# shenwei356/bio

Measured on AMD Instinct MI355X. Metric: Gbases/s hashed (k=21 ntHash + minimizer), higher is better.
Workload: dtype u64

## Files before the change

bio_amd/csrc/biosketch.hip:

```cpp
#include "host_internal.hpp"
#include "kernels_host.hpp"

extern "C" int bsk_abi_version(void) { return BSK_ABI_VERSION; }

extern "C" const char *bsk_err_name(int e) {
    switch (e) {
        case BSK_OK: return "ok";
        case BSK_ERR_INVALID_K: return "ErrInvalidK";
        case BSK_ERR_EMPTY_SEQ: return "ErrEmptySeq";
        case BSK_ERR_SHORT_SEQ: return "ErrShortSeq";
        case BSK_ERR_ILLEGAL_BASE: return "ErrIllegalBase";
        case BSK_ERR_K_TOO_LARGE: return "ErrKTooLarge";
        case BSK_ERR_INVALID_M: return "ErrInvalidM";
        case BSK_ERR_INVALID_SCALE: return "ErrInvalidScale";
        case BSK_ERR_INVALID_S: return "ErrInvalidS";
        case BSK_ERR_INVALID_W: return "ErrInvalidW";
        case BSK_ERR_BUF_NIL: return "ErrBufNil";
        case BSK_ERR_BUF_NOT_EMPTY: return "ErrBufNotEmpty";
        case BSK_ERR_ARG: return "bad argument";
        case BSK_ERR_NOMEM: return "out of memory";
        case BSK_ERR_DEVICE: return "device error";
        case BSK_ERR_UNSUPPORTED: return "unsupported";
        case BSK_ERR_NO_DEVICE: return "no gfx950 device";
        case BSK_ERR_IO: return "fastx: cannot open or read the file";
// ... 168 lines not shown
    }
    if (hipMemcpyAsync(b->d_odd, b->odd->data(), b->odd->size() * sizeof(u64), hipMemcpyHostToDevice, ctx->stream) != hipSuccess) {
        (void)hipGetLastError();
        (void)hipFree(b->d_odd);
        b->d_odd = nullptr;
    }
}

u64 pad_words(u32 maxlen) { return (u64)maxlen / 16 + kMaxPrefetchWords + 1; }
u32 env_u32(const char *name, u32 dflt) {
    const char *v = getenv(name);
    return v && *v ? (u32)strtoul(v, nullptr, 10) : dflt;
}
u32 min_tile_min(const bsk_ctx *ctx) { return ctx->opt.tile_min ? ctx->opt.tile_min : std::min<u32>(64u, 16u * (BSK_NT_FAST_WORDS - 2)); }
void BskOpts::load() {
    auto on = [](const char *n) { return getenv(n) != nullptr; };
    force_generic = on("BSK_FORCE_GENERIC");
    no_mixed = on("BSK_NO_MIXED");
    no_dense = on("BSK_NO_DENSE");
    no_pk = on("BSK_NO_PK");
    no_ring = on("BSK_NO_RING");
    no_pkd = on("BSK_NO_PKD");
    no_side_early = on("BSK_NO_SIDE_EARLY");
    no_side_dense = on("BSK_NO_SIDE_DENSE");
    no_bin = on("BSK_NO_BIN");
    no_bin_early = on("BSK_NO_BIN_EARLY");
    compact = on("BSK_COMPACT");
    ring = on("BSK_RING");
    ring_max = env_u32("BSK_RING_MAX", 0);
    ring_sel10 = env_u32("BSK_RING_SEL10", 0);
    bin_min = env_u32("BSK_BIN_MIN", 1024);
    no_class = on("BSK_NO_CLASS");
    syn_sel = on("BSK_SYN_SEL");
    class_min = env_u32("BSK_CLASS_MIN", 16384);
    class_force = on("BSK_CLASS_FORCE");
    class_view = on("BSK_CLASS_VIEW");
    no_syn_pf = on("BSK_NO_SYN_PF");
    pf_density = env_u32("BSK_PF_DENSITY", 0);
    no_syn_long = on("BSK_NO_SYN_LONG");
    syn_margin = (int)env_u32("BSK_SYN_MARGIN", (u32)PlannerTable::syn_margin_rows + 64) - 64;
    no_tiles = on("BSK_NO_TILES");
    no_spare = on("BSK_NO_SPARE");
    no_tile_cache = on("BSK_NO_TILE_CACHE");
    tile_dense = on("BSK_TILE_DENSE");
    no_tile_defer = on("BSK_NO_TILE_DEFER");
    no_group_gather = on("BSK_NO_GROUP_GATHER");
// ... 120 lines not shown
    }
    b->device_bytes = nbytes + 64 + (n + 1) * 8;
    if (alphabet == BSK_ALPHA_DNA) {
        const bool wide = maxlen >= (1u << 24);
        if (ctx->h_refs_cap < n + 1) {
            if (ctx->h_refs) (void)hipHostFree(ctx->h_refs);
            ctx->h_refs = nullptr;
            ctx->h_refs_cap = 0;
            const size_t want = (n + 1) + (n + 1) / 4 + 64;
            BCHK(hipHostMalloc(&ctx->h_refs, want * 8));
            ctx->h_refs_cap = want;
        }
        u64 *const desc = ctx->h_refs;
        std::vector<u64> llen(wide ? n : 0);
        u64 w = 0;
        LenHist *hist = (!uniform && !wide && n) ? new (std::nothrow) LenHist() : nullptr;
        for (u64 r = 0; r < n; ++r) {
            u64 L = offsets[r + 1] - offsets[r];
            desc[r] = wide ? w : ((w << 24) | L);
            if (wide) llen[r] = L;
            if (hist) hist->add(L);
            w += (L + 15) / 16;
        }
        delete b->hist;
        b->hist = hist;
        collect_odd(b, n, [&](u64 r) { return offsets[r + 1] - offsets[r]; });
        upload_odd(ctx, b);
        b->n_words = w;
        const u64 alloc_words = w + pad_words(maxlen);
        BCHK(take((void **)&b->words, &b->c_words, alloc_words * sizeof(u32), donor ? (void **)&donor->words : nullptr, donor ? &donor->c_words : nullptr));
        if (wide) BCHK(hipMalloc(&b->fw, (n ? n : 1) * sizeof(u64)));
        else BCHK(take((void **)&b->desc, &b->c_desc, (n ? n : 1) * sizeof(u64), donor ? (void **)&donor->desc : nullptr, donor ? &donor->c_desc : nullptr));
        if (wide) {
            BCHK(hipMalloc(&b->llen, n * sizeof(u64)));
            BCHK(hipMemcpyAsync(b->llen, llen.data(), n * sizeof(u64), hipMemcpyHostToDevice, ctx->stream));
        }
        BCHK(take((void **)&b->rflags, &b->c_rflags, n ? n : 1, donor ? (void **)&donor->rflags : nullptr, donor ? &donor->c_rflags : nullptr));
        BCHK(hipMemsetAsync(b->words, 0, alloc_words * sizeof(u32), ctx->stream));
        BCHK(hipMemsetAsync(b->rflags, 0, n ? n : 1, ctx->stream));
        if (n) BCHK(hipMemcpyAsync(wide ? b->fw : b->desc, desc, n * sizeof(u64), hipMemcpyHostToDevice, ctx->stream));
        BCHK(hipMemsetAsync(ctx->d_ticket, 0, 2 * sizeof(u32), ctx->stream));
        if (maxlen > min_tile_min(ctx) && w) {
            BCHK(hipMalloc(&b->wbits, ((w + 31) / 32) * sizeof(u32)));
            BCHK(hipMemsetAsync(b->wbits, 0, ((w + 31) / 32) * sizeof(u32), ctx->stream));
        }
        if (n && w) {
// ... 35 lines not shown
                                    bsk_batch **out) {
    return batch_from_ascii_impl(ctx, bytes, offsets, n, alphabet, nullptr, out);
}

extern "C" int bsk_batch_refill_ascii(bsk_ctx *ctx, bsk_batch **batch, const uint8_t *bytes, const uint64_t *offsets, uint64_t n, int alphabet) {
    if (!ctx || !batch) return fail_arg(ctx, "bsk_batch_refill_ascii: null argument");
    bsk_batch *old = *batch;
    if (old && (old->ctx != ctx || old->alias)) return fail_arg(ctx, "bsk_batch_refill_ascii: the batch belongs to another context");
    *batch = nullptr;
    return batch_from_ascii_impl(ctx, bytes, offsets, n, alphabet, old, batch);
}

static int batch_from_packed_impl(bsk_ctx *ctx, const uint32_t *words, uint64_t n_words, const uint64_t *desc, uint64_t n, bsk_batch *donor,
                                  bsk_batch **out) {
    struct DonorGuard {
        bsk_batch *d;
        ~DonorGuard() { if (d) bsk_batch_destroy(d); }
    } donor_guard{donor};
    if (!ctx || !out || (n && !desc) || (n_words && !words)) return fail_arg(ctx, "bsk_batch_from_packed: null argument");
    *out = nullptr;
    HIPCHK(ctx, hipSetDevice(ctx->device));
    u32 maxlen = 0;
    u64 nb = 0;
    bool uniform = true;
    std::unique_ptr<LenHist> hist;
    for (u64 r = 0; r < n; ++r) {
        u64 L = desc[r] & 0xffffffULL, w0 = desc[r] >> 24;
        if (w0 + (L + 15) / 16 > n_words) return fail_arg(ctx, "desc points outside words[]");
        maxlen = std::max<u32>(maxlen, (u32)L);
        nb += L;
        if (L != (desc[0] & 0xffffffULL) && uniform) {
            uniform = false;
            hist.reset(new (std::nothrow) LenHist());
            if (hist) {
                hist->cnt[LenHist::bucket(desc[0] & 0xffffffULL)] = r;
                hist->bases[LenHist::bucket(desc[0] & 0xffffffULL)] = r * (desc[0] & 0xffffffULL);
                hist->hi[LenHist::bucket(desc[0] & 0xffffffULL)] = (u32)(desc[0] & 0xffffffULL);
                hist->lo[LenHist::bucket(desc[0] & 0xffffffULL)] = (u32)(desc[0] & 0xffffffULL);
            }
        }
        if (hist) hist->add(L);
    }
    bsk_batch *b = new (std::nothrow) bsk_batch();
    if (!b) return BSK_ERR_NOMEM;
    b->hist = hist.release();
    collect_odd(b, n, [&](u64 r) { return desc[r] & 0xffffffULL; });
    upload_odd(ctx, b);
    b->ctx = ctx;
    b->alphabet = BSK_ALPHA_DNA;
    b->n = n;
    b->n_bases = nb;
    b->n_words = n_words;
    b->maxlen = maxlen;
    b->uniform_len = (n && uniform) ? maxlen : 0;
    const u64 alloc_words = n_words + pad_words(maxlen);
    auto take = [&](void **dst, size_t *cap_dst, size_t need, void **src, size_t *cap_src) -> hipError_t {
        if (donor && *src && *cap_src >= need) {
            *dst = *src;
            *cap_dst = *cap_src;
            *src = nullptr;
            *cap_src = 0;
            return hipSuccess;
        }
        const size_t want = donor ? need + need / 8 + 256 : need;
        const hipError_t e2 = hipMalloc(dst, want ? want : 1);
        if (e2 == hipSuccess) *cap_dst = want;
        return e2;
    };
    if (donor) {
        std::swap(b->bdesc, donor->bdesc);
        std::swap(b->c_bdesc, donor->c_bdesc);
        std::swap(b->bflags, donor->bflags);
        std::swap(b->c_bflags, donor->c_bflags);
        std::swap(b->spare_ascii, donor->spare_ascii);
        std::swap(b->spare_aoff, donor->spare_aoff);
        if (donor->ascii && !b->spare_ascii) {
            b->spare_ascii = donor->ascii;
// ... 37 lines not shown
    if (!ctx || !batch) return fail_arg(ctx, "bsk_batch_refill_packed: null argument");
    bsk_batch *old = *batch;
    if (old && (old->ctx != ctx || old->alias)) return fail_arg(ctx, "bsk_batch_refill_packed: the batch belongs to another context");
    *batch = nullptr;
    return batch_from_packed_impl(ctx, words, n_words, desc, n, old, batch);
}

extern "C" int bsk_batch_synth(bsk_ctx *ctx, int alphabet, uint64_t n, uint32_t len, uint64_t seed, bsk_batch **out) {
    if (!ctx || !out) return fail_arg(ctx, "bsk_batch_synth: null argument");
    if (len == 0 || len >= (1u << 24) || n == 0) return fail_arg(ctx, "bsk_batch_synth: bad n/len");
    *out = nullptr;
    HIPCHK(ctx, hipSetDevice(ctx->device));
    bsk_batch *b = new (std::nothrow) bsk_batch();
    if (!b) return BSK_ERR_NOMEM;
    b->ctx = ctx;
    b->alphabet = alphabet;
    b->n = n;
    b->n_bases = n * len;
    b->maxlen = len;
    b->uniform_len = len;
    hipError_t e = hipSuccess;
    if (alphabet == BSK_ALPHA_DNA) {
        const u32 wpr = (len + 15) / 16;
        b->n_words = n * wpr;
        const u64 alloc_words = b->n_words + pad_words(len);
        if ((e = hipMalloc(&b->words, alloc_words * 4)) == hipSuccess && (e = hipMalloc(&b->desc, n * 8)) == hipSuccess &&
            (e = hipMalloc(&b->rflags, n)) == hipSuccess &&
            (e = hipMemsetAsync(b->words + b->n_words, 0, pad_words(len) * 4, ctx->stream)) == hipSuccess) {
            hipLaunchKernelGGL(k_synth_dna, dim3(grid_for(ctx, b->n_words, 256)), dim3(256), 0, ctx->stream, b->words, b->desc,
                               b->rflags, n, len, wpr, seed);
            e = hipGetLastError();
        }
        b->device_bytes = alloc_words * 4 + n * 9;
    } else if (alphabet == BSK_ALPHA_PROTEIN) {
        if ((e = hipMalloc(&b->ascii, n * len + BSK_ASCII_PAD)) == hipSuccess && (e = hipMalloc(&b->aoff, (n + 1) * 8)) == hipSuccess) {
            hipLaunchKernelGGL(k_synth_protein, dim3(grid_for(ctx, n * len, 256)), dim3(256), 0, ctx->stream, b->ascii, b->aoff, n,
                               len, seed);
            e = hipGetLastError();
        }
        b->device_bytes = n * len + 64 + (n + 1) * 8;
    } else {
        delete b;
        return fail_arg(ctx, "bad alphabet");
    }
    if (e == hipSuccess) e = hipStreamSynchronize(ctx->stream);
    if (e != hipSuccess) {
// ... 712 lines not shown
```

bio_amd/csrc/classes.hip:

```cpp
#include "host_internal.hpp"
#include "kernels_host.hpp"

void class_set_free(ClassSet *cs) {
    if (!cs) return;
    for (auto &pt : cs->parts) {
        if (pt.res) bsk_result_release(pt.res);
        if (pt.sub) bsk_batch_destroy(pt.sub);
    }
    if (cs->view) bsk_batch_destroy(cs->view);
    delete cs;
}
extern "C" int bsk_result_class_plan(const bsk_result *r, int *n_parts, float *build_ms) {
    if (!r) return BSK_ERR_ARG;
    if (n_parts) *n_parts = r->classes ? (int)r->classes->parts.size() : 0;
    if (build_ms) *build_ms = r->classes ? r->classes->build_ms : 0.0f;
    return BSK_OK;
}

int launch_parts(bsk_ctx *ctx, ClassSet *cs, const bsk_params *p, bsk_result *res, bool tiled) {
    bsk_ctx *side = ctx->side;
    for (auto &pt : cs->parts) {
        if (pt.tiled != tiled) continue;
        const u64 base = res->cap + pt.off;
        if (base + pt.extent > res->alloc_cap) {
// ... 255 lines not shown
        (void)hipEventRecord(e1, ctx->stream);
        (void)hipEventSynchronize(e1);
        (void)hipEventElapsedTime(&cs->build_ms, e0, e1);
    }
    if (e0) (void)hipEventDestroy(e0);
    if (e1) (void)hipEventDestroy(e1);
    if (!cs->view) cs->view = new (std::nothrow) bsk_batch();
    if (!cs->view) return BSK_ERR_NOMEM;
    {
        bsk_batch *v = cs->view;
        u64 *bd = v->bdesc;
        u8 *bf = v->bflags;
        const size_t cbd = v->c_bdesc, cbf = v->c_bflags;
        *v = *b;
        v->hist = nullptr;
        v->borrowed = true;
        v->odd = nullptr;
        v->d_odd = nullptr;
        if (!masked) v->desc = view;
        v->side_maxlen = b->maxlen;
        v->maxlen = bk.hi;
        v->n_bases = pretend ? (u64)pretend * b->n : bk.bases;
        v->uniform_len = pretend;
        v->bdesc = bd;
        v->bflags = bf;
        v->c_bdesc = cbd;
        v->c_bflags = cbf;
        v->bin_gran = 0;
        v->bin_lo = 0;
        v->bin_early = false;
        v->spare_ascii = nullptr;
        v->spare_aoff = nullptr;
    }
    cs->n = b->n;
    cs->n_bases = b->n_bases;
    cs->maxlen = b->maxlen;
    cs->desc = b->desc;
    cs->words = b->words;
    cs->blo = cuts[(size_t)bulk].lo;
    cs->bhi = cuts[(size_t)bulk].hi;
    return BSK_OK;
}

static void class_plan_names(bsk_result *res, const ClassSet *cs) {
    size_t at = strlen(res->plan);
    for (const auto &pt : cs->parts) {
// ... 147 lines not shown
```

bio_amd/csrc/fast_dispatch.hpp:

```cpp
#pragma once
#include <hip/hip_runtime.h>

#include "kernels_generic.hpp"

#define BSK_FAST_CAP 32
#define BSK_SYN_CAP 28
#define BSK_ASCII_PAD 1024

namespace bsk {
bool fast_minimizer_supported(int w);
int fast_minimizer_blocks_per_cu(int w);
void fast_minimizer_launch(int w, int grid, hipStream_t stream, const KArgs &a);
bool dense_minimizer_supported(int w);
int dense_minimizer_blocks_per_cu(int w);
void dense_minimizer_launch(int w, int grid, hipStream_t stream, const KArgs &a);
void dense_minimizer_ascii_launch(int w, int grid, hipStream_t stream, const KArgs &a);
int dense_minimizer_ascii_blocks_per_cu(int w);

bool pk_minimizer_supported(int w);
int pk_minimizer_blocks_per_cu(int w);
u32 pk_minimizer_short_bases();
void pk_minimizer_launch(int w, bool long_reads, int grid, hipStream_t stream, const KArgs &a);
void pk_minimizer_list_launch(int w, int grid, hipStream_t stream, const KArgs &a);

bool pkd_minimizer_supported(int w);
int pkd_minimizer_blocks_per_cu(int w);
void pkd_minimizer_launch(int w, int grid, hipStream_t stream, const KArgs &a);

bool ring_minimizer_supported(int w);
int ring_minimizer_blocks_per_cu(int w);
u32 ring_minimizer_short_bases();
void ring_minimizer_launch(int w, bool long_reads, int grid, hipStream_t stream, const KArgs &a);

bool seg_minimizer_supported(int w);
int seg_minimizer_blocks_per_cu(int w);
void seg_minimizer_launch(int w, int grid, hipStream_t stream, const KArgs &a);

void wpr_minimizer_launch(int grid, hipStream_t stream, const KArgs &a);
int wpr_minimizer_blocks_per_cu();

bool fast_syncmer_supported(int k, int s);
int fast_syncmer_blocks_per_cu(int w);
void fast_syncmer_launch(int w, int grid, hipStream_t stream, const KArgs &a);
void fast_syncmer_ascii_launch(int w, int grid, hipStream_t stream, const KArgs &a);
// ... 42 lines not shown
```

bio_amd/csrc/host_types.hpp:

```cpp
#pragma once
#include <hip/hip_runtime.h>

#include <cstdio>
#include <string>
#include <vector>

#include "biosketch.h"
#include "device_common.hpp"

struct BskOpts {
    bool force_generic = false, no_mixed = false, no_dense = false, no_pk = false, no_ring = false, no_pkd = false, no_side_early = false, no_side_dense = false, ring = false, no_bin = false, no_bin_early = false, compact = false, no_spare = false, no_tiles = false, no_tile_cache = false, no_tile_defer = false, tile_dense = false, no_group_gather = false, timing = false,
         no_fused_translate = false, sets_no_small = false;
    int syn_margin = 2;
    u32 test_overflow = 0;
    bool no_syn_long = false;
    u32 pf_density = 0;
    bool no_syn_pf = false;
    bool syn_sel = false;
    bool no_class = false;
    u32 class_min = 16384;
    bool class_view = false;
    bool class_force = false;
    u32 wpr = 0, seg = 0, dense_min = 21 , ring_max = 0, ring_sel10 = 0 , bin_min = 1024, waves_per_cu = 0, tile_min = 0, tile_pos = 0;
    void load();
};

enum PoolSlot {
    SLOT_TILE_START = 0, SLOT_TILE_DESC = 1, SLOT_TILE_ADESC = 2, SLOT_TILE_SEQ = 3, SLOT_TILE_SHIFT = 4, SLOT_TILE_KEEP = 5, SLOT_TILE_FLAGS = 6, SLOT_TILE_SEQ_FLAGS = 7,
    SLOT_TILE_SEQ_BAD = 8, SLOT_TILE_EXCL = 9,
    SLOT_SETS_OFFS = 0, SLOT_SETS_PART = 1, SLOT_SETS_VALUES = 2, SLOT_SETS_UCOUNT = 3, SLOT_SETS_SORTED = 5, SLOT_SETS_HEAD = 6, SLOT_SETS_KEEP = 7, SLOT_SETS_POS = 8,
    SLOT_SETS_TMP = 9,
    SLOT_SEARCH_QUERY = 10, SLOT_SEARCH_RANGES = 11, SLOT_SEARCH_STAGE = 15, SLOT_SEARCH_LARGE = 30, SLOT_SEARCH_SORT_TMP = 31,
    SLOT_FETCH_OFFS = 12, SLOT_FETCH_HASH = 13, SLOT_FETCH_POS = 14,
    SLOT_COMPACT_OFFS = 16,
// ... 68 lines not shown
    }
    static int bucket(u64 L) {
        if (L < 1024) return (int)(L >> 4);
        const int lg = 63 - __builtin_clzll(L);
        return 64 + 4 * (lg - 10) + (int)((L >> (lg - 2)) & 3);
    }
    void add(u64 L) {
        const int i = bucket(L);
        cnt[i]++;
        bases[i] += L;
        if ((u32)L > hi[i]) hi[i] = (u32)L;
        if ((u32)L < lo[i]) lo[i] = (u32)L;
    }
};

struct bsk_batch {
    bsk_ctx *ctx = nullptr;
    int alphabet = BSK_ALPHA_DNA;
    int pairs = BSK_ALPHA_DNA;
    u64 n = 0, n_bases = 0, n_words = 0, n_nonacgt = 0;
    u32 maxlen = 0;
    u32 side_maxlen = 0;
    u32 uniform_len = 0;
    u32 *words = nullptr;
    u64 *desc = nullptr;
    u64 *fw = nullptr;
    u64 *llen = nullptr;
    u64 *adesc = nullptr;
    bool alias = false;
    bool borrowed = false;
    LenHist *hist = nullptr;
    std::vector<u64> *odd = nullptr;
    u64 *d_odd = nullptr;
    int modal_bucket = -1;
    u32 *wbits = nullptr;
    u32 *subset = nullptr;
    u64 nsub = 0;
    u8 *rflags = nullptr;
    mutable u64 *bdesc = nullptr;
    mutable u8 *bflags = nullptr;
    mutable u32 bin_gran = 0, bin_lo = 0;
    mutable bool bin_early = false;
    mutable size_t c_bdesc = 0, c_bflags = 0;
    u8 *ascii = nullptr;
    u64 *aoff = nullptr;
    u64 device_bytes = 0;
// ... 82 lines not shown
```

bio_amd/csrc/kernels_generic.hpp:

```cpp
#pragma once
#include "device_common.hpp"
#include "biosketch.h"

namespace bsk {

struct KArgs {
    const u32 *words;
    const u64 *desc;
    const u8 *ascii;
    const u64 *aoff;
    const u64 *adesc;
    const u8 *rflags;
    u64 n;
    u32 nunits;
    int kind, k, w, s, canonical, circ_ext, m, scale;
    u64 *refs;
    u8 *status;
    u64 *hash;
    u32 *pos;
    u64 cap;
    u32 *ticket;
    u32 fixcap;
    u32 *rlist;
    u64 *fixlist;
    u64 *lookback;
    u64 *total;
    u64 *ring_h;
    u32 *ring_p;
    u32 ring_w;
    u32 uniform_len;
    u64 slab_read;
    u64 list_slab;
    u32 unit_rows;
    u64 ovf_base;
    u64 ovf_cap;
    const u32 *subset;
    u64 nsub;
    u64 out_base;
    int inplace;
    int frame;
    const u8 *lut;
    int pairs;
    int one_strand;
    u32 *sel_mask, *sel_cnt, *sel_utot;
    u64 *sel_ubase, *sel_lookback;
    u32 sel_nb;
    const u64 *tkeep, *tshift;
    u32 cls_lo, cls_hi, cls_pretend;
    u32 tk;
    u32 list_grid;
    u32 len_mask;
    u32 binned;
};

__device__ __forceinline__ void list_append(const KArgs &a, u32 *list, u32 seg, u32 &cur, u64 redo, int lane, u64 r) {
    const u32 at = cur + __builtin_amdgcn_mbcnt_hi((u32)(redo >> 32), __builtin_amdgcn_mbcnt_lo((u32)redo, 0));
    if ((redo >> lane) & 1) {
        if (at < seg) list[a.list_grid + blockIdx.x * seg + at] = (u32)r;
        else atomicOr(&a.ticket[1], 2u);
    }
    cur += (u32)__builtin_popcountll(redo);
}
__device__ __forceinline__ void list_close(u32 *list, u32 seg, u32 cur, int lane) {
    if (lane == 0) list[blockIdx.x] = cur < seg ? cur : seg;
}

__device__ __forceinline__ u64 desc_len(const KArgs &a, u64 d) {
    u64 L = d & (u64)a.len_mask;
    if (a.cls_hi) L = (L >= (u64)a.cls_lo && L <= (u64)a.cls_hi) ? L : (u64)a.cls_pretend;
    return L;
}
#ifdef BSK_BIN_NOSCATTER
// ... 392 lines not shown
```

bio_amd/csrc/kernels_pk.hpp:

```cpp
#pragma once
#include <utility>

#include "kernels_fast.hpp"

namespace bsk {

template <int... Is, class F>
__device__ __forceinline__ void pk_unroll_impl(std::integer_sequence<int, Is...>, F &&f) {
    (f(std::integral_constant<int, Is>{}), ...);
}
template <int N, class F>
__device__ __forceinline__ void pk_unroll(F &&f) {
    pk_unroll_impl(std::make_integer_sequence<int, N>{}, f);
}

#ifndef BSK_PK_ROWS
#define BSK_PK_ROWS 58
#endif
struct PkLds {
    static constexpr int PR = BSK_PK_ROWS;
    static constexpr int ROW = 33;
    static constexpr int TAB = 0;
    static constexpr int TAB2 = 320;
    static constexpr int NHEADS = (32 * (PR - 1)) / 64 + 2;
// ... 33 lines not shown
        if (at != 0xffffffffu) *reinterpret_cast<LDSQ u32x4 *>(ldsq + at) = row;
        wave_sync_lds();
    }
};

template <int W>
struct PkCfg {
    static constexpr int XC = W > 12 ? 4 : W;
};

#define PKNW 16
typedef u32 u32x16 __attribute__((ext_vector_type(16)));
struct PkWords {
    u32x4 a, b, c, d;
};
__device__ __forceinline__ PkWords pk_load_words(const u32 *p) {
    PkWords r;
    asm volatile("global_load_dwordx4 %0, %4, off\n\tglobal_load_dwordx4 %1, %4, off offset:16\n\t"
                 "global_load_dwordx4 %2, %4, off offset:32\n\tglobal_load_dwordx4 %3, %4, off offset:48"
                 : "=&v"(r.a), "=&v"(r.b), "=&v"(r.c), "=&v"(r.d)
                 : "v"(p));
    return r;
}
__device__ __forceinline__ u64 pk_load_u64(const u64 *p) {
    u64 r;
    asm volatile("global_load_dwordx2 %0, %1, off" : "=&v"(r) : "v"(p));
    return r;
}
__device__ __forceinline__ void pk_wait_loads(u64 &d0, u64 &d1) { asm volatile("s_waitcnt vmcnt(0)" : "+v"(d0), "+v"(d1)::"memory"); }
__device__ __forceinline__ void pk_wait_loads(PkWords &p) { asm volatile("s_waitcnt vmcnt(0)" : "+v"(p.a), "+v"(p.b), "+v"(p.c), "+v"(p.d)::"memory"); }
__device__ __forceinline__ void pk_ticket_async(u32 *ticket, u32 &t) {
    u64 ex;
    asm volatile("s_mov_b64 %1, exec\n\ts_mov_b64 exec, 1\n\tglobal_atomic_add %0, %2, %3, off sc0\n\ts_mov_b64 exec, %1"
                 : "+v"(t), "=&s"(ex)
                 : "v"(ticket), "v"(1u)
                 : "memory");
}
__device__ __forceinline__ void pk_wait_loads(PkWords &p, u64 &d0, u32 &f, u32 &t) {
    asm volatile("s_waitcnt vmcnt(0)" : "+v"(p.a), "+v"(p.b), "+v"(p.c), "+v"(p.d), "+v"(d0), "+v"(f), "+v"(t)::"memory");
}
__device__ __forceinline__ u32 pk_load_u8(const u8 *p) {
    u32 r;
    asm volatile("global_load_ubyte %0, %1, off" : "=&v"(r) : "v"(p));
    return r;
}
template <int W, bool LONG, class LY_ = PkLds, bool RINGM = false, bool SELM = false>
struct PkMin {
    typedef LY_ LY;
    const u32 *__restrict__ w;
    LDSQ char *lds;
    int k, lane;
    u32 nk;
    u32 fl, fh_, rl, rh_;
    u32 S[W];
    u64 H[W];
    u32 SB[W];
    u32 P, bm, tmin;
    u32 nsel;
    u32 slot, spare;
    u32 glo, gspan;
    u32 c8000;
    int sstep;
// ... 411 lines not shown
#ifndef PK_NOHASHST
                __builtin_nontemporal_store(hv[j], &gh[t]);
#else
                asm volatile("" ::"v"(hv[j]));
#endif
#ifndef PK_NOPOSST
                __builtin_nontemporal_store(POS2 ? __builtin_amdgcn_alignbit(pv[j], pv[j], 1) : pv[j] & 0x80007fffu, &gp[t]);
#else
                asm volatile("" ::"v"(pv[j]));
#endif
            }
#endif
        }
    };
    u32 t0 = 0;
    for (; t0 + 64 * U <= T; t0 += 64 * U) trip(t0, std::false_type{});
    if (t0 < T) trip(t0, std::true_type{});
    wave_sync_lds();
}

#ifndef PK_TICKET
#define PK_TICKET 8u
#endif
template <int W, bool LONG>
__global__ __launch_bounds__(64, 2) void k_minimizer_pk(KArgs a) {
    typedef PkLds LY;
    __shared__ __attribute__((aligned(16))) char lds[LY::TOTAL];
    LDSQ char *const ldsq = (LDSQ char *)lds;
    const int lane = lane_id();
    PkTabs tabs;
    tabs.init(a.k, lane);
#ifdef PK_STAGGER
    for (u32 i = (((blockIdx.x * 2654435761u) >> 24) * (u32)PK_STAGGER) >> 8; i; --i) __builtin_amdgcn_s_sleep(32);
#endif
    const u64 slab = (u64)64 * BSK_FAST_CAP;
    const u32 col8 = (u32)(lane & 31) * 8u;
    constexpr u32 RB = (u32)(LY::ROW * 8);
    const u32 top = (u32)(LY::PR - 1) * RB + col8;
    u64 d_n1 = 0, d_cur = 0;
    PkWords pw_cur = {{0, 0, 0, 0}, {0, 0, 0, 0}, {0, 0, 0, 0}, {0, 0, 0, 0}};
    bool have = false;
    const u32 lseg = a.fixcap / a.list_grid;
    u32 lcur = 0;
    const u32 tku = a.tk ? a.tk : PK_TICKET;
    const bool ahead = tku >= 3u;
    u32 tv = 0;
    u32 nt = ~0u;
    for (u32 unit = next_ticket(a.ticket, lane) * tku, uend = unit + tku; unit < a.nunits; ++unit, ({
             if (unit == uend) {
                 unit = ahead ? nt : next_ticket(a.ticket, lane) * tku;
                 uend = unit + tku;
             }
         })) {
        const u64 r = (u64)unit * 64 + lane;
        const u64 u2 = (!ahead || unit + 2u < uend) ? (u64)unit + 2u : (u64)nt + (unit + 2u - uend);
        const bool nxt = unit + 1 != uend ? unit + 1 < a.nunits : ahead && nt < a.nunits;
        const bool ask = ahead && unit + 3u == uend;
        const u64 rmax = a.n - 1;
        if (!have) {
            d_cur = pk_load_u64(a.desc + (r < rmax ? r : rmax));
            d_n1 = pk_load_u64(a.desc + (r + 64 < rmax ? r + 64 : rmax));
            pk_wait_loads(d_cur, d_n1);
            pw_cur = pk_load_words(a.words + (d_cur >> 24));
            pk_wait_loads(pw_cur);
        }
        PkWords pw_n1 = pk_load_words(a.words + (d_n1 >> 24));
        const u64 r2 = u2 * 64 + lane;
        u64 d_n2 = pk_load_u64(a.desc + (r2 < rmax ? r2 : rmax));
        u32 rfl = pk_load_u8(a.rflags ? a.rflags + (r < rmax ? r : rmax) : reinterpret_cast<const u8 *>(a.desc));
        if (ask) pk_ticket_async(a.ticket, tv);
        const u64 d = d_cur;
        const PkWords pw = pw_cur;
        const u64 off = d >> 24, L = desc_len(a, d);
        const u64 ro = out_index(a, r, d);
        const bool ok = r < a.n && L >= (u64)a.circ_ext && (L - (u64)a.circ_ext) + 1 >= (u64)a.k + (u64)W;
        const u32 nk = ok ? (u32)(L - a.k + 1) : 0u;
        const u32 nk_max = wave_max_u32(nk);
        const u32 nk_min = ~wave_max_u32(~(ok ? nk : 0xffffffffu));
        u32 cnt = 0, tmin_lane = 0xffffffffu;
        if (nk_max) {
            tabs.write(ldsq);
            PkMin<W, LONG> pm;
            pm.w = a.words + off;
            pm.set_words(pw);
            pm.lds = ldsq;
            pm.k = a.k;
            pm.lane = lane;
            pm.nk = nk;
            const u32 spare = (u32)LY::PR * RB + col8;
            pm.run(nk_max, ok, nk_min, !ok ? spare : lane < 32 ? col8 : top, !ok ? 0 : lane < 32 ? (int)RB : -(int)RB, col8);
            if (ok) cnt = (lane < 32 ? pm.slot - col8 : top - pm.slot) / RB;
            tmin_lane = pm.tmin;
        }
        pk_wait_loads(pw_n1, d_n2, rfl, tv);
        if (ask) nt = (u32)__builtin_amdgcn_readfirstlane((int)tv) * tku;
        d_cur = d_n1;
        pw_cur = pw_n1;
        d_n1 = d_n2;
        have = nxt;
        const u32 cnt_pair = cnt + (u32)__builtin_amdgcn_ds_bpermute((lane ^ 32) * 4, (int)cnt);
        u64 bad = __builtin_amdgcn_ballot_w64(cnt_pair >= (u32)LY::PR);
        u64 tied = __builtin_amdgcn_ballot_w64(ok && tmin_lane < 32u);
#if defined(PK_NOSTAGE) || defined(PK_NOTIE) || defined(PK_NOTAB) || defined(PK_NOCOPY) || defined(PK_NOSTORE) || defined(PK_NOFB)
        bad = 0;
        tied = 0;
#endif
        const u64 redo = bad | tied;
        if (redo) {
            list_append(a, a.rlist, lseg, lcur, redo, lane, r);
            if ((redo >> lane) & 1) cnt = 0;
        }
        const u32 incl = wave_incl_scan_u32(cnt, lane);
        const u32 excl = incl - cnt;
        const u32 T = wave_bcast_u32(incl, 63);
        const u64 base = (u64)unit * slab;
#ifndef PK_NOCOPY
#ifndef PK_CU
#define PK_CU 8
// ... 21 lines not shown
    hipError_t e = hipErrorInvalidValue;
    switch (w) {
#define X(WW) \
    case WW: e = hipOccupancyMaxActiveBlocksPerMultiprocessor(&nb, k_minimizer_pk<WW, false>, 64, 0); break;
        BSK_PK_WS(X)
#undef X
        default: break;
    }
    if (e != hipSuccess || nb < 1) {
        (void)hipGetLastError();
        nb = 1;
    }
    return nb;
}
void pk_minimizer_list_launch(int w, int grid, hipStream_t stream, const KArgs &a) {
    switch (w) {
#define X(WW) \
    case WW: hipLaunchKernelGGL((k_minimizer_dense<WW, true>), dim3(grid), dim3(64), 0, stream, a); break;
        BSK_PK_WS(X)
#undef X
        default: break;
    }
}
void pk_minimizer_launch(int w, bool long_reads, int grid, hipStream_t stream, const KArgs &a) {
    switch (w) {
#define X(WW)                                                                                               \
    case WW:                                                                                                \
        if (long_reads) {                                                                                   \
            hipLaunchKernelGGL((k_minimizer_pk<WW, true>), dim3(grid), dim3(64), 0, stream, a);             \
        } else {                                                                                            \
            hipLaunchKernelGGL((k_minimizer_pk<WW, false>), dim3(grid), dim3(64), 0, stream, a);            \
        }                                                                                                   \
        hipLaunchKernelGGL((k_minimizer_dense<WW, true>), dim3(grid), dim3(64), 0, stream, a);              \
        break;
        BSK_PK_WS(X)
#undef X
        default: break;
    }
}
#endif

}
```

bio_amd/csrc/launch.hip:

```cpp
#include "host_internal.hpp"
#include "kernels_host.hpp"

int launch(bsk_ctx *ctx, const bsk_batch *b, const bsk_params *p, bsk_result *res, int circ_ext, const Plan &pl,
                  hipEvent_t ev0, hipEvent_t ev1) {
    if (pl.nunits == 0) return BSK_OK;
    ClassSet *const cs = (ctx->cls && b == ctx->cls->view) ? ctx->cls : nullptr;
    if (cs) {
        if (ev0) HIPCHK(ctx, hipEventRecord(ev0, ctx->stream));
        HIPCHK(ctx, hipMemsetAsync(ctx->d_ticket + 16, 0, sizeof(u32), ctx->stream));
        HIPCHK(ctx, hipEventRecord(ctx->ev_adopted, ctx->stream));
        HIPCHK(ctx, hipStreamWaitEvent(ctx->side->stream, ctx->ev_adopted, 0));
        const int trc = launch_parts(ctx, cs, p, res, true);
        if (trc != BSK_OK) return trc;
        bool any_tiled = false;
        for (auto &pt : cs->parts) any_tiled |= pt.tiled && pt.n;
        if (any_tiled) {
            HIPCHK(ctx, hipEventRecord(ctx->ev_tiled, ctx->side->stream));
            HIPCHK(ctx, hipStreamWaitEvent(ctx->stream, ctx->ev_tiled, 0));
        }
        const int prc = launch_parts(ctx, cs, p, res, false);
        if (prc != BSK_OK) return prc;
    }
    KArgs a;
    memset(&a, 0, sizeof a);
    a.words = b->words;
    a.desc = b->desc;
    a.ascii = b->ascii;
    a.aoff = b->aoff;
    a.adesc = b->adesc;
    a.rflags = b->rflags;
    a.n = b->n;
    a.nunits = pl.nunits;
    a.kind = p->kind;
    a.k = p->k;
    a.w = p->w;
    a.s = p->s;
    a.m = p->m;
    a.scale = p->scale;
    a.canonical = p->canonical > 0 ? 1 : 0;
    a.one_strand = p->canonical < 0 ? 1 : 0;
    a.pairs = b->pairs;
    a.circ_ext = circ_ext;
    a.uniform_len = b->uniform_len;
    a.refs = res->refs;
    a.status = res->status;
    a.hash = res->hash;
    a.pos = res->pos;
    a.cap = res->main_cap ? res->main_cap : res->cap;
    a.ovf_base = pl.slab_total;
    a.slab_read = pl.slab_read;
    a.ovf_cap = res->ovf_cap;
    a.ticket = ctx->d_ticket;
    a.total = ctx->d_total;
    a.ring_w = pl.ring_w;
    a.len_mask = 0xffffffu;
    {
        const u32 own = (pl.which == K_MIN_PKD || pl.which == K_MIN_DENSE || pl.which == K_PROT_MIN_FAST) ? 4u : 8u;
        const u64 waves = (u64)std::max(pl.grid, 1);
        a.tk = 0;
        if ((pl.which == K_MIN_PK || pl.which == K_MIN_PKD || pl.which == K_MIN_RING || pl.which == K_SYN_PK || pl.which == K_MIN_FAST || pl.which == K_MIN_DENSE || pl.which == K_SYN_FAST ||
             pl.which == K_PROT_MIN_FAST) && (u64)pl.nunits < waves * own)
            a.tk = (u32)std::max<u64>(1, ((u64)pl.nunits + waves - 1) / waves);
    }
    if (cs && cs->masked) {
        a.cls_lo = cs->blo;
        a.cls_hi = cs->bhi;
        a.cls_pretend = cs->pretend;
    }
    if (pl.bin_gran) {
        const int brc = ensure_binned(ctx, b, (u32)((p->kind == BSK_SYNCMER ? p->s : p->k) - 1), pl.bin_gran, a.cls_lo, a.cls_hi, a.cls_pretend);
        if (brc != BSK_OK) return brc;
        a.desc = b->bdesc;
        a.rflags = b->rflags ? b->bflags : nullptr;
        a.len_mask = 0xfffu;
        a.binned = 1;
    }
    const bool lists = pl.which == K_SYN_PK || pl.which == K_MIN_PK || pl.which == K_MIN_RING || pl.which == K_SYN_SEL || pl.which == K_MIN_PKD;
    const u64 fixcap = lists ? syn_pk_fixcap(b->n, pl.grid) : 0;
    int rc = ensure_scratch(ctx, std::max<u32>(lists ? (u32)((fixcap + (u64)pl.grid) / 2 + 2) : pl.slab ? 1 : pl.nunits, pl.mixed ? pl.side_nunits : 0), pl.ring_entries);
    if (rc != BSK_OK) return rc;
    a.lookback = ctx->d_lookback;
    a.fixlist = ctx->d_lookback;
    a.fixcap = (u32)fixcap;
    a.list_grid = (u32)pl.grid;
    a.rlist = reinterpret_cast<u32 *>(ctx->d_lookback);
// ... 5 lines not shown
    if (pl.which == K_MIN_PKD) {
        const u64 nwin_max = b->maxlen + 2 > (u32)(p->k + p->w) ? (u64)b->maxlen - p->k - p->w + 2 : 1;
        a.list_slab = (nwin_max + 15) & ~(u64)15;
    }
    a.ring_h = ctx->d_ring_h;
    a.ring_p = ctx->d_ring_p;
    HIPCHK(ctx, hipMemsetAsync(ctx->d_ticket, 0, 8 * sizeof(u32), ctx->stream));
    HIPCHK(ctx, hipMemsetAsync(ctx->d_total, 0, 4 * sizeof(u64), ctx->stream));
    if (!pl.slab) HIPCHK(ctx, hipMemsetAsync(ctx->d_lookback, 0, (size_t)pl.nunits * sizeof(u64), ctx->stream));
    if (ev0 && !cs) HIPCHK(ctx, hipEventRecord(ev0, ctx->stream));
    auto side_launch = [&](hipStream_t st, u64 *lookback, u64 *refs_to, u8 *status_to) -> int {
        KArgs sd = a;
        sd.desc = b->desc;
        sd.rflags = b->rflags;
        sd.len_mask = 0xffffffu;
        sd.binned = 0;
        sd.cls_lo = sd.cls_hi = sd.cls_pretend = 0;
        sd.subset = b->subset;
        sd.nsub = b->nsub;
        sd.nunits = pl.side_nunits;
        sd.out_base = res->main_cap;
        sd.cap = res->cap;
        sd.uniform_len = 0;
        sd.inplace = !kind_has_pos(p->kind);
        sd.ticket = ctx->d_ticket + 2;
        sd.total = ctx->d_total + 2;
        sd.ring_w = pl.side_ring_w;
        sd.lookback = lookback;
        sd.refs = refs_to;
        sd.status = status_to;
        HIPCHK(ctx, hipMemsetAsync(lookback, 0, (size_t)pl.side_nunits * sizeof(u64), st));
        switch (pl.side_which) {
            case K_MIN_GEN_A: hipLaunchKernelGGL(k_minimizer_generic<1>, dim3(pl.side_grid), dim3(64), 0, st, sd); break;
            case K_MIN_DENSE_A:
                sd.slab_read = pl.side_slab;
                dense_minimizer_ascii_launch(p->w, pl.side_grid, st, sd);
                break;
            case K_SYN_FAST_A:
                sd.ovf_base = res->main_cap + (u64)pl.side_nunits * 64 * pl.side_slab;
                sd.ovf_cap = res->cap > sd.ovf_base ? res->cap - sd.ovf_base : 0;
                fast_syncmer_ascii_launch(p->k - p->s, pl.side_grid, st, sd);
                break;
            case K_NT_A: hipLaunchKernelGGL(k_nthash_stream<1>, dim3(pl.side_grid), dim3(64), 0, st, sd); break;
            case K_SYN_A: hipLaunchKernelGGL(k_syncmer<1>, dim3(pl.side_grid), dim3(64), 0, st, sd); break;
            case K_KMER_A: hipLaunchKernelGGL(k_kmer<1>, dim3(pl.side_grid), dim3(64), 0, st, sd); break;
            case K_SIM_A: hipLaunchKernelGGL(k_simhash<1>, dim3(pl.side_grid), dim3(64), 0, st, sd); break;
// ... 4 lines not shown
    bool side_early = false;
    u64 *side_refs = nullptr;
    u8 *side_status = nullptr;
    if (pl.mixed && kind_has_pos(p->kind) && !ctx->opt.no_side_early && side_ctx(ctx)) {
        bsk_ctx *sc = ctx->side;
        if (ensure_scratch(sc, pl.side_nunits, 0) == BSK_OK && ctx_pool(ctx, SLOT_SIDE_REFS, (size_t)b->n * 8, &side_refs) == hipSuccess &&
            ctx_pool(ctx, SLOT_SIDE_STATUS, (size_t)b->n, &side_status) == hipSuccess) {
            HIPCHK(ctx, hipEventRecord(ctx->ev_mix0, ctx->stream));
            HIPCHK(ctx, hipStreamWaitEvent(sc->stream, ctx->ev_mix0, 0));
            const int src = side_launch(sc->stream, sc->d_lookback, side_refs, side_status);
            if (src != BSK_OK) return src;
            side_early = true;
        } else {
            (void)hipGetLastError();
        }
    }
    const bool main_moot = side_early && !cs && b->nsub == b->n && (pl.side_which == K_MIN_DENSE_A || pl.side_which == K_SYN_FAST_A);
    if (!main_moot) switch (pl.which) {
        case K_MIN_GEN_P: hipLaunchKernelGGL(k_minimizer_generic<0>, dim3(pl.grid), dim3(64), 0, ctx->stream, a); break;
        case K_MIN_GEN_A: hipLaunchKernelGGL(k_minimizer_generic<1>, dim3(pl.grid), dim3(64), 0, ctx->stream, a); break;
        case K_NT_P: hipLaunchKernelGGL(k_nthash_stream<0>, dim3(pl.grid), dim3(64), 0, ctx->stream, a); break;
        case K_NT_A: hipLaunchKernelGGL(k_nthash_stream<1>, dim3(pl.grid), dim3(64), 0, ctx->stream, a); break;
        case K_MIN_FAST: fast_minimizer_launch(pl.fast_w, pl.grid, ctx->stream, a); break;
        case K_MIN_PK: pk_minimizer_launch(pl.fast_w, b->maxlen > pk_minimizer_short_bases(), pl.grid, ctx->stream, a); break;
        case K_MIN_RING: ring_minimizer_launch(pl.fast_w, b->maxlen > ring_minimizer_short_bases(), pl.grid, ctx->stream, a); break;
        case K_MIN_DENSE: dense_minimizer_launch(pl.fast_w, pl.grid, ctx->stream, a); break;
        case K_MIN_PKD: pkd_minimizer_launch(pl.fast_w, pl.grid, ctx->stream, a); break;
        case K_MIN_DENSE_A:
        case K_SYN_FAST_A: break;
#ifdef BSK_EXPERIMENTS
        case K_MIN_SEG: seg_minimizer_launch(pl.fast_w, pl.grid, ctx->stream, a); break;
        case K_MIN_WPR: wpr_minimizer_launch(pl.grid, ctx->stream, a); break;
#else
        case K_MIN_SEG:
        case K_MIN_WPR: break;
#endif
        case K_SYN_P: hipLaunchKernelGGL(k_syncmer<0>, dim3(pl.grid), dim3(64), 0, ctx->stream, a); break;
        case K_SYN_A: hipLaunchKernelGGL(k_syncmer<1>, dim3(pl.grid), dim3(64), 0, ctx->stream, a); break;
        case K_KMER_P: hipLaunchKernelGGL(k_kmer<0>, dim3(pl.grid), dim3(64), 0, ctx->stream, a); break;
        case K_KMER_A: hipLaunchKernelGGL(k_kmer<1>, dim3(pl.grid), dim3(64), 0, ctx->stream, a); break;
        case K_SIM_P: hipLaunchKernelGGL(k_simhash<0>, dim3(pl.grid), dim3(64), 0, ctx->stream, a); break;
        case K_SIM_A: hipLaunchKernelGGL(k_simhash<1>, dim3(pl.grid), dim3(64), 0, ctx->stream, a); break;
        case K_PROT_HASH: hipLaunchKernelGGL(k_prot_hash, dim3(pl.grid), dim3(64), 0, ctx->stream, a); break;
        case K_PROT_MIN: hipLaunchKernelGGL(k_prot_minimizer, dim3(pl.grid), dim3(64), 0, ctx->stream, a); break;
        case K_SYN_FAST: fast_syncmer_launch(pl.fast_w, pl.grid, ctx->stream, a); break;
        case K_SYN_PK:
            if (pl.syn_fused) pf_syncmer_launch(pl.fast_w, pl.syn_long, pl.grid, std::min(pl.grid, ctx->cus * 8), ctx->stream, a);
// ... 362 lines not shown
```

Baseline: 1258.

## Add fixed-stride uniform-length path to pk minimizer and shrink tail ticket size

Adds a template variant of the pk minimizer kernel for uniform-length, evenly strided reads. It computes word addresses directly from the row index, which drops the per-read descriptor loads and the wave reductions for k-mer counts. It also loads only as many 16-byte quads as the stride needs. Separately, the ticket scheduler hands out smaller chunks in a final tail region to balance the end of the work across waves. The costs are extra template instantiations, new host bookkeeping of word stride, and a more complex ticket-to-unit mapping.

```diff
diff --git a/bio_amd/csrc/biosketch.hip b/bio_amd/csrc/biosketch.hip
--- a/bio_amd/csrc/biosketch.hip
+++ b/bio_amd/csrc/biosketch.hip
@@ -214,6 +214,9 @@
     no_ring = on("BSK_NO_RING");
     no_pkd = on("BSK_NO_PKD");
     no_side_early = on("BSK_NO_SIDE_EARLY");
+    pk_tail = env_u32("BSK_PK_TAIL", 1);
+    pk_small = std::min(std::max(env_u32("BSK_PK_SMALL", 3), 3u), 8u);
+    pk_no_uniform = on("BSK_PK_NO_UNIFORM");
     no_side_dense = on("BSK_NO_SIDE_DENSE");
     no_bin = on("BSK_NO_BIN");
     no_bin_early = on("BSK_NO_BIN_EARLY");
@@ -380,6 +383,7 @@
             if (hist) hist->add(L);
             w += (L + 15) / 16;
         }
+        if (b->uniform_len && !wide) b->word_stride = (maxlen + 15) / 16;
         delete b->hist;
         b->hist = hist;
         collect_odd(b, n, [&](u64 r) { return offsets[r + 1] - offsets[r]; });
@@ -461,11 +465,13 @@
     HIPCHK(ctx, hipSetDevice(ctx->device));
     u32 maxlen = 0;
     u64 nb = 0;
-    bool uniform = true;
+    bool uniform = true, strided = true;
+    const u64 wpr0 = n ? ((desc[0] & 0xffffffULL) + 15) / 16 : 0;
     std::unique_ptr<LenHist> hist;
     for (u64 r = 0; r < n; ++r) {
         u64 L = desc[r] & 0xffffffULL, w0 = desc[r] >> 24;
         if (w0 + (L + 15) / 16 > n_words) return fail_arg(ctx, "desc points outside words[]");
+        if (w0 != r * wpr0) strided = false;
         maxlen = std::max<u32>(maxlen, (u32)L);
         nb += L;
         if (L != (desc[0] & 0xffffffULL) && uniform) {
@@ -492,6 +498,7 @@
     b->n_words = n_words;
     b->maxlen = maxlen;
     b->uniform_len = (n && uniform) ? maxlen : 0;
+    b->word_stride = (b->uniform_len && strided) ? (u32)wpr0 : 0;
     const u64 alloc_words = n_words + pad_words(maxlen);
     auto take = [&](void **dst, size_t *cap_dst, size_t need, void **src, size_t *cap_src) -> hipError_t {
         if (donor && *src && *cap_src >= need) {
@@ -575,6 +582,7 @@
     hipError_t e = hipSuccess;
     if (alphabet == BSK_ALPHA_DNA) {
         const u32 wpr = (len + 15) / 16;
+        b->word_stride = wpr;
         b->n_words = n * wpr;
         const u64 alloc_words = b->n_words + pad_words(len);
         if ((e = hipMalloc(&b->words, alloc_words * 4)) == hipSuccess && (e = hipMalloc(&b->desc, n * 8)) == hipSuccess &&
diff --git a/bio_amd/csrc/classes.hip b/bio_amd/csrc/classes.hip
--- a/bio_amd/csrc/classes.hip
+++ b/bio_amd/csrc/classes.hip
@@ -301,6 +301,7 @@
         v->maxlen = bk.hi;
         v->n_bases = pretend ? (u64)pretend * b->n : bk.bases;
         v->uniform_len = pretend;
+        v->word_stride = 0;
         v->bdesc = bd;
         v->bflags = bf;
         v->c_bdesc = cbd;
diff --git a/bio_amd/csrc/fast_dispatch.hpp b/bio_amd/csrc/fast_dispatch.hpp
--- a/bio_amd/csrc/fast_dispatch.hpp
+++ b/bio_amd/csrc/fast_dispatch.hpp
@@ -20,6 +20,7 @@
 bool pk_minimizer_supported(int w);
 int pk_minimizer_blocks_per_cu(int w);
 u32 pk_minimizer_short_bases();
+bool pk_minimizer_uniform(bool long_reads, const KArgs &a);
 void pk_minimizer_launch(int w, bool long_reads, int grid, hipStream_t stream, const KArgs &a);
 void pk_minimizer_list_launch(int w, int grid, hipStream_t stream, const KArgs &a);
 
diff --git a/bio_amd/csrc/host_types.hpp b/bio_amd/csrc/host_types.hpp
--- a/bio_amd/csrc/host_types.hpp
+++ b/bio_amd/csrc/host_types.hpp
@@ -9,7 +9,8 @@
 #include "device_common.hpp"
 
 struct BskOpts {
-    bool force_generic = false, no_mixed = false, no_dense = false, no_pk = false, no_ring = false, no_pkd = false, no_side_early = false, no_side_dense = false, ring = false, no_bin = false, no_bin_early = false, compact = false, no_spare = false, no_tiles = false, no_tile_cache = false, no_tile_defer = false, tile_dense = false, no_group_gather = false, timing = false,
+    u32 pk_tail = 1, pk_small = 3;
+    bool force_generic = false, no_mixed = false, no_dense = false, no_pk = false, no_ring = false, no_pkd = false, no_side_early = false, pk_no_uniform = false, no_side_dense = false, ring = false, no_bin = false, no_bin_early = false, compact = false, no_spare = false, no_tiles = false, no_tile_cache = false, no_tile_defer = false, tile_dense = false, no_group_gather = false, timing = false,
          no_fused_translate = false, sets_no_small = false;
     int syn_margin = 2;
     u32 test_overflow = 0;
@@ -124,6 +125,7 @@
     u32 maxlen = 0;
     u32 side_maxlen = 0;
     u32 uniform_len = 0;
+    u32 word_stride = 0;
     u32 *words = nullptr;
     u64 *desc = nullptr;
     u64 *fw = nullptr;
diff --git a/bio_amd/csrc/kernels_generic.hpp b/bio_amd/csrc/kernels_generic.hpp
--- a/bio_amd/csrc/kernels_generic.hpp
+++ b/bio_amd/csrc/kernels_generic.hpp
@@ -29,6 +29,7 @@
     u32 *ring_p;
     u32 ring_w;
     u32 uniform_len;
+    u32 uni_stride;
     u64 slab_read;
     u64 list_slab;
     u32 unit_rows;
@@ -48,6 +49,7 @@
     const u64 *tkeep, *tshift;
     u32 cls_lo, cls_hi, cls_pretend;
     u32 tk;
+    u32 tk_t0, tk_small;
     u32 list_grid;
     u32 len_mask;
     u32 binned;
diff --git a/bio_amd/csrc/kernels_pk.hpp b/bio_amd/csrc/kernels_pk.hpp
--- a/bio_amd/csrc/kernels_pk.hpp
+++ b/bio_amd/csrc/kernels_pk.hpp
@@ -79,6 +79,22 @@
                  : "v"(p));
     return r;
 }
+__device__ __forceinline__ PkWords pk_load_words_n(const u32 *p, u32 nq) {
+    PkWords r;
+    asm volatile("global_load_dwordx4 %0, %4, off\n\t"
+                 "s_cmp_lt_u32 %5, 3\n\ts_cbranch_scc1 .Lpkw_low%=\n\t"
+                 "global_load_dwordx4 %1, %4, off offset:16\n\tglobal_load_dwordx4 %2, %4, off offset:32\n\t"
+                 "s_cmp_lt_u32 %5, 4\n\ts_cbranch_scc1 .Lpkw_end%=\n\t"
+                 "global_load_dwordx4 %3, %4, off offset:48\n\ts_branch .Lpkw_end%=\n"
+                 ".Lpkw_low%=:\n\t"
+                 "s_cmp_lt_u32 %5, 2\n\ts_cbranch_scc1 .Lpkw_end%=\n\t"
+                 "global_load_dwordx4 %1, %4, off offset:16\n"
+                 ".Lpkw_end%=:"
+                 : "=&v"(r.a), "=&v"(r.b), "=&v"(r.c), "=&v"(r.d)
+                 : "v"(p), "s"(nq)
+                 : "scc");
+    return r;
+}
 __device__ __forceinline__ u64 pk_load_u64(const u64 *p) {
     u64 r;
     asm volatile("global_load_dwordx2 %0, %1, off" : "=&v"(r) : "v"(p));
@@ -95,6 +111,9 @@
 }
 __device__ __forceinline__ void pk_wait_loads(PkWords &p, u64 &d0, u32 &f, u32 &t) {
     asm volatile("s_waitcnt vmcnt(0)" : "+v"(p.a), "+v"(p.b), "+v"(p.c), "+v"(p.d), "+v"(d0), "+v"(f), "+v"(t)::"memory");
+}
+__device__ __forceinline__ void pk_wait_loads(PkWords &p, u32 &f, u32 &t) {
+    asm volatile("s_waitcnt vmcnt(0)" : "+v"(p.a), "+v"(p.b), "+v"(p.c), "+v"(p.d), "+v"(f), "+v"(t)::"memory");
 }
 __device__ __forceinline__ u32 pk_load_u8(const u8 *p) {
     u32 r;
@@ -552,8 +571,9 @@
 #ifndef PK_TICKET
 #define PK_TICKET 8u
 #endif
-template <int W, bool LONG>
+template <int W, bool LONG, bool UNI = false>
 __global__ __launch_bounds__(64, 2) void k_minimizer_pk(KArgs a) {
+    static_assert(!(UNI && LONG), "k_minimizer_pk: the fixed-length form keeps the whole read in registers");
     typedef PkLds LY;
     __shared__ __attribute__((aligned(16))) char lds[LY::TOTAL];
     LDSQ char *const ldsq = (LDSQ char *)lds;
@@ -573,13 +593,20 @@
     const u32 lseg = a.fixcap / a.list_grid;
     u32 lcur = 0;
     const u32 tku = a.tk ? a.tk : PK_TICKET;
+    const u32 t0s = a.tk_small ? a.tk_t0 : 0xffffffffu, u0s = a.tk_small ? a.tk_t0 * tku : 0xffffffffu;
+    const u32 tsm = a.tk_small ? a.tk_small : tku;
+    auto ticket_unit = [&](u32 t) { return t < t0s ? t * tku : u0s + (t - t0s) * tsm; };
+    auto ticket_end = [&](u32 first) { return first + (first < u0s ? tku : tsm); };
+    const u32 uL = a.uniform_len;
+    const u32 unk = (UNI && uL >= (u32)a.circ_ext && (uL - (u32)a.circ_ext) + 1u >= (u32)a.k + (u32)W) ? uL - (u32)a.k + 1u : 0u;
+    const u32 unq = a.uni_stride / 4u + 1u < 4u ? a.uni_stride / 4u + 1u : 4u;
     const bool ahead = tku >= 3u;
     u32 tv = 0;
     u32 nt = ~0u;
-    for (u32 unit = next_ticket(a.ticket, lane) * tku, uend = unit + tku; unit < a.nunits; ++unit, ({
+    for (u32 unit = ticket_unit(next_ticket(a.ticket, lane)), uend = ticket_end(unit); unit < a.nunits; ++unit, ({
              if (unit == uend) {
-                 unit = ahead ? nt : next_ticket(a.ticket, lane) * tku;
-                 uend = unit + tku;
+                 unit = ahead ? nt : ticket_unit(next_ticket(a.ticket, lane));
+                 uend = ticket_end(unit);
              }
          })) {
         const u64 r = (u64)unit * 64 + lane;
@@ -587,26 +614,49 @@
         const bool nxt = unit + 1 != uend ? unit + 1 < a.nunits : ahead && nt < a.nunits;
         const bool ask = ahead && unit + 3u == uend;
         const u64 rmax = a.n - 1;
-        if (!have) {
+        if constexpr (UNI) {
+            if (!have) {
+                pw_cur = pk_load_words_n(a.words + (r < rmax ? r : rmax) * (u64)a.uni_stride, unq);
+                pk_wait_loads(pw_cur);
+            }
+        } else if (!have) {
             d_cur = pk_load_u64(a.desc + (r < rmax ? r : rmax));
             d_n1 = pk_load_u64(a.desc + (r + 64 < rmax ? r + 64 : rmax));
             pk_wait_loads(d_cur, d_n1);
             pw_cur = pk_load_words(a.words + (d_cur >> 24));
             pk_wait_loads(pw_cur);
         }
-        PkWords pw_n1 = pk_load_words(a.words + (d_n1 >> 24));
-        const u64 r2 = u2 * 64 + lane;
-        u64 d_n2 = pk_load_u64(a.desc + (r2 < rmax ? r2 : rmax));
+        PkWords pw_n1;
+        u64 d_n2 = 0;
+        if constexpr (UNI) {
+            const u64 r1 = ((!ahead || unit + 1u < uend) ? (u64)unit + 1u : (u64)nt) * 64 + lane;
+            pw_n1 = pk_load_words_n(a.words + (r1 < rmax ? r1 : rmax) * (u64)a.uni_stride, unq);
+        } else {
+            pw_n1 = pk_load_words(a.words + (d_n1 >> 24));
+            const u64 r2 = u2 * 64 + lane;
+            d_n2 = pk_load_u64(a.desc + (r2 < rmax ? r2 : rmax));
+        }
         u32 rfl = pk_load_u8(a.rflags ? a.rflags + (r < rmax ? r : rmax) : reinterpret_cast<const u8 *>(a.desc));
         if (ask) pk_ticket_async(a.ticket, tv);
         const u64 d = d_cur;
         const PkWords pw = pw_cur;
-        const u64 off = d >> 24, L = desc_len(a, d);
-        const u64 ro = out_index(a, r, d);
-        const bool ok = r < a.n && L >= (u64)a.circ_ext && (L - (u64)a.circ_ext) + 1 >= (u64)a.k + (u64)W;
-        const u32 nk = ok ? (u32)(L - a.k + 1) : 0u;
-        const u32 nk_max = wave_max_u32(nk);
-        const u32 nk_min = ~wave_max_u32(~(ok ? nk : 0xffffffffu));
+        u64 off, ro;
+        bool ok;
+        u32 nk, nk_max, nk_min;
+        if constexpr (UNI) {
+            off = 0;
+            ro = r;
+            ok = r < a.n && unk != 0u;
+            nk = nk_max = nk_min = unk;
+        } else {
+            const u64 L = desc_len(a, d);
+            off = d >> 24;
+            ro = out_index(a, r, d);
+            ok = r < a.n && L >= (u64)a.circ_ext && (L - (u64)a.circ_ext) + 1 >= (u64)a.k + (u64)W;
+            nk = ok ? (u32)(L - a.k + 1) : 0u;
+            nk_max = wave_max_u32(nk);
+            nk_min = ~wave_max_u32(~(ok ? nk : 0xffffffffu));
+        }
         u32 cnt = 0, tmin_lane = 0xffffffffu;
         if (nk_max) {
             tabs.write(ldsq);
@@ -622,8 +672,9 @@
             if (ok) cnt = (lane < 32 ? pm.slot - col8 : top - pm.slot) / RB;
             tmin_lane = pm.tmin;
         }
-        pk_wait_loads(pw_n1, d_n2, rfl, tv);
-        if (ask) nt = (u32)__builtin_amdgcn_readfirstlane((int)tv) * tku;
+        if constexpr (UNI) pk_wait_loads(pw_n1, rfl, tv);
+        else pk_wait_loads(pw_n1, d_n2, rfl, tv);
+        if (ask) nt = ticket_unit((u32)__builtin_amdgcn_readfirstlane((int)tv));
         d_cur = d_n1;
         pw_cur = pw_n1;
         d_n1 = d_n2;
@@ -691,12 +742,16 @@
         default: break;
     }
 }
+bool pk_minimizer_uniform(bool long_reads, const KArgs &a) { return !long_reads && a.uni_stride && a.uniform_len && !a.cls_hi && !a.binned && !a.subset; }
 void pk_minimizer_launch(int w, bool long_reads, int grid, hipStream_t stream, const KArgs &a) {
+    const bool uni = pk_minimizer_uniform(long_reads, a);
     switch (w) {
 #define X(WW)                                                                                               \
     case WW:                                                                                                \
         if (long_reads) {                                                                                   \
             hipLaunchKernelGGL((k_minimizer_pk<WW, true>), dim3(grid), dim3(64), 0, stream, a);             \
+        } else if (uni) {                                                                                   \
+            hipLaunchKernelGGL((k_minimizer_pk<WW, false, true>), dim3(grid), dim3(64), 0, stream, a);      \
         } else {                                                                                            \
             hipLaunchKernelGGL((k_minimizer_pk<WW, false>), dim3(grid), dim3(64), 0, stream, a);            \
         }                                                                                                   \
diff --git a/bio_amd/csrc/launch.hip b/bio_amd/csrc/launch.hip
--- a/bio_amd/csrc/launch.hip
+++ b/bio_amd/csrc/launch.hip
@@ -42,6 +42,7 @@
     a.pairs = b->pairs;
     a.circ_ext = circ_ext;
     a.uniform_len = b->uniform_len;
+    a.uni_stride = (b->alphabet == BSK_ALPHA_DNA && !pl.mixed && !ctx->opt.pk_no_uniform) ? b->word_stride : 0;
     a.refs = res->refs;
     a.status = res->status;
     a.hash = res->hash;
@@ -61,6 +62,11 @@
         if ((pl.which == K_MIN_PK || pl.which == K_MIN_PKD || pl.which == K_MIN_RING || pl.which == K_SYN_PK || pl.which == K_MIN_FAST || pl.which == K_MIN_DENSE || pl.which == K_SYN_FAST ||
              pl.which == K_PROT_MIN_FAST) && (u64)pl.nunits < waves * own)
             a.tk = (u32)std::max<u64>(1, ((u64)pl.nunits + waves - 1) / waves);
+        if (pl.which == K_MIN_PK && !a.tk && ctx->opt.pk_tail) {
+            const u64 region = std::min<u64>((u64)ctx->opt.pk_tail * waves * own, pl.nunits);
+            a.tk_t0 = (u32)(((u64)pl.nunits - region) / own);
+            a.tk_small = ctx->opt.pk_small;
+        }
     }
     if (cs && cs->masked) {
         a.cls_lo = cs->blo;
@@ -112,6 +118,7 @@
         sd.out_base = res->main_cap;
         sd.cap = res->cap;
         sd.uniform_len = 0;
+        sd.uni_stride = 0;
         sd.inplace = !kind_has_pos(p->kind);
         sd.ticket = ctx->d_ticket + 2;
         sd.total = ctx->d_total + 2;
@@ -162,7 +169,12 @@
         case K_NT_P: hipLaunchKernelGGL(k_nthash_stream<0>, dim3(pl.grid), dim3(64), 0, ctx->stream, a); break;
         case K_NT_A: hipLaunchKernelGGL(k_nthash_stream<1>, dim3(pl.grid), dim3(64), 0, ctx->stream, a); break;
         case K_MIN_FAST: fast_minimizer_launch(pl.fast_w, pl.grid, ctx->stream, a); break;
-        case K_MIN_PK: pk_minimizer_launch(pl.fast_w, b->maxlen > pk_minimizer_short_bases(), pl.grid, ctx->stream, a); break;
+        case K_MIN_PK:
+            if (ctx->opt.timing)
+                fprintf(stderr, "[bsk] k_minimizer_pk: %s form, tk %u, tk_t0 %u, tk_small %u\n", pk_minimizer_uniform(b->maxlen > pk_minimizer_short_bases(), a) ? "fixed-length" : "general", a.tk, a.tk_t0,
+                        a.tk_small);
+            pk_minimizer_launch(pl.fast_w, b->maxlen > pk_minimizer_short_bases(), pl.grid, ctx->stream, a);
+            break;
         case K_MIN_RING: ring_minimizer_launch(pl.fast_w, b->maxlen > ring_minimizer_short_bases(), pl.grid, ctx->stream, a); break;
         case K_MIN_DENSE: dense_minimizer_launch(pl.fast_w, pl.grid, ctx->stream, a); break;
         case K_MIN_PKD: pkd_minimizer_launch(pl.fast_w, pl.grid, ctx->stream, a); break;
```

Result: faster. 1277 (median of 6 runs) (+1.5%).
